# QEDProtocol/plonky2.5

Hardware: NVIDIA B200
Metric: commit Melem/s (2^20x135 LDE+Poseidon Merkle) (higher is better)
Workload: dtype u64 (Goldilocks field, integer + exact fp64 limb arithmetic)

## Files before the change

### plonky2.5_b200/csrc/gl_commit.cu

```cuda
#include <cuda_runtime.h>
#include <nvtx3/nvToolsExt.h>

#include <cstdio>
#include <algorithm>
#include <exception>
#include <cstring>
#include <cstdlib>
#include <condition_variable>
#include <map>
#include <thread>
#include <utility>
#include <memory>
#include <mutex>
#include <set>
#include <string>
#include <vector>

#include "../../include/gl_commit.h"
#include "fri.cuh"
#include "gates.cuh"
#include "merkle.cuh"
#include "microbench.cuh"
#include "ntt.cuh"
#include "ntt2.cuh"
#include "openings.cuh"
#include "peer_sync.cuh"
#include "permutation.cuh"

#ifndef LEAF_BLOCK
#define LEAF_BLOCK 128
#endif

namespace {

struct GlError {
    int code;
    std::string msg;
};

struct NvtxRange {
    explicit NvtxRange(const char* name) { nvtxRangePushA(name); }
    ~NvtxRange() { nvtxRangePop(); }
    NvtxRange(const NvtxRange&) = delete;
    NvtxRange& operator=(const NvtxRange&) = delete;
};


#define GL_THROW(code, ...)                              \
    do {                                                 \
        char _b[512];                                    \
        snprintf(_b, sizeof _b, __VA_ARGS__);            \
        throw GlError{code, _b};                         \
    } while (0)

#define CUDA_CHECK(expr)                                                                                   \
    do {                                                                                                   \
        cudaError_t _e = (expr);                                                                           \
        if (_e != cudaSuccess) {                                                                           \
            int _c = (_e == cudaErrorMemoryAllocation) ? GL_ERR_OOM : GL_ERR_CUDA;                         \
            GL_THROW(_c, "%s failed: %s (%s:%d)", #expr, cudaGetErrorString(_e), __FILE__, __LINE__);      \
        }                                                                                                  \
    } while (0)

struct DevPool {
    std::mutex mu;
    std::multimap<std::pair<int, size_t>, uint64_t*> free_list;
    size_t cached_words = 0;
    static DevPool& get() { static DevPool p; return p; }
    uint64_t* take(int dev, size_t words) {
        std::lock_guard<std::mutex> lk(mu);
        auto it = free_list.find({dev, words});
        if (it == free_list.end()) return nullptr;
        uint64_t* p = it->second;
        free_list.erase(it);
        cached_words -= words;
        return p;
    }
    void give(int dev, size_t words, uint64_t* p) {
        std::lock_guard<std::mutex> lk(mu);
        free_list.insert({{dev, words}, p});
        cached_words += words;
    }
    void trim(int dev) {
        std::lock_guard<std::mutex> lk(mu);
        for (auto it = free_list.begin(); it != free_list.end();) {
            if (it->first.first == dev) { cudaFree(it->second); cached_words -= it->first.second; it = free_list.erase(it); }
            else ++it;
        }
    }
};

struct DevBuf {
    uint64_t* p = nullptr;
    size_t words = 0;
    int dev = -1;
    void ensure(size_t w) {
        if (w <= words) return;
        release();
        if (w == 0) w = 1;
        CUDA_CHECK(cudaGetDevice(&dev));
        p = DevPool::get().take(dev, w);
        if (!p) {
            cudaError_t e = cudaMalloc(&p, w * sizeof(uint64_t));
            if (e == cudaErrorMemoryAllocation) {
                cudaGetLastError();
                DevPool::get().trim(dev);
                e = cudaMalloc(&p, w * sizeof(uint64_t));
            }
            if (e != cudaSuccess) { p = nullptr; CUDA_CHECK(e); }
        }
        words = w;
    }
    void release() {
        if (p && std::uncaught_exceptions() > 0) cudaDeviceSynchronize();
        if (p) DevPool::get().give(dev, words, p);
        p = nullptr;
        words = 0;
    }
    ~DevBuf() { release(); }
    DevBuf() = default;
    DevBuf(const DevBuf&) = delete;
    DevBuf& operator=(const DevBuf&) = delete;
};

inline uint32_t round_up(uint32_t x, uint32_t m) { return (x + m - 1) / m * m; }
inline uint32_t log2_exact(uint64_t n) {
    uint32_t l = 0;
    while ((1ULL << l) < n) l++;
    return l;
}
inline uint32_t h_bitrev(uint32_t x, uint32_t bits) {
    uint32_t r = 0;
    for (uint32_t i = 0; i < bits; i++) { r = (r << 1) | (x & 1); x >>= 1; }
    return r;
}

std::vector<uint32_t> plan_passes(uint32_t n, uint32_t max_a = 10) {
    std::vector<uint32_t> v;
    if (n < 3) return v;
    uint32_t k = (n + max_a - 1) / max_a, base = n / k, rem = n % k;
    for (uint32_t i = 0; i < k; i++) v.push_back(base + (i < rem ? 1 : 0));
    return v;
}

struct CosetTable {
    uint64_t g = 1;
    DevBuf F;
};

struct Tree {
    uint64_t n_leaves = 0;
    uint32_t leaf_len = 0, pitch = 0, cap_height = 0, degree_log = 0, rate_bits = 0;
    DevBuf leaves, digests, coeffs, d_cap;
    bool has_coeffs = false;
    std::vector<uint64_t> cap;
    Tree(uint64_t n_leaves_, uint32_t leaf_len_, uint32_t pitch_, uint32_t cap_height_)
        : n_leaves(n_leaves_), leaf_len(leaf_len_), pitch(pitch_), cap_height(cap_height_), cap(4ULL << cap_height_) {
        leaves.ensure(n_leaves * pitch);
        digests.ensure(n_digests() * 4);
        d_cap.ensure(4ULL << cap_height);
    }
    uint64_t n_digests() const { return 2 * (n_leaves - (1ULL << cap_height)); }
};

struct Fri {
    uint64_t len = 0;
    uint32_t rate_bits = 0, cap_height = 0;
    uint64_t shift = gl::COSET_SHIFT;
    uint32_t last_arity_bits = 0;
    DevBuf coeffs, values, tmp;
    Fri(uint64_t len_, uint32_t rate_bits_, uint32_t cap_height_) : len(len_), rate_bits(rate_bits_), cap_height(cap_height_) {
        coeffs.ensure(2 * len); values.ensure(2 * len); tmp.ensure(2 * len);
    }
};

struct Quotient {
    gl_handle wires = 0;
    uint64_t n_rows = 0;
    uint32_t n_challenges = 0;
    DevBuf acc, powers;
};

struct Openings {
    uint32_t log_n = 0;
    DevBuf final_poly, comp, refs, pw;
};

template <class T>
struct Handles {
    const char* kind;
    std::map<gl_handle, std::unique_ptr<T>> live;
    gl_handle put(gl_ctx* c, std::unique_ptr<T> obj);
    T* get(gl_handle h) const;
    void drop(gl_ctx* c, gl_handle h);
};

}

struct gl_ctx {
    int device = 0;
    cudaStream_t stream = nullptr;
    std::mutex mu;
    std::string err;
    std::map<uint32_t, std::unique_ptr<DevBuf>> roots;
    std::map<uint32_t, std::unique_ptr<DevBuf>> pass_roots;
    std::map<uint64_t, std::unique_ptr<std::vector<CosetTable>>> lde_tables;
    std::map<std::pair<uint64_t, uint32_t>, std::unique_ptr<CosetTable>> coset_cache;
    size_t coset_cache_words = 0;
    DevBuf in_stage, vals, scratch, hash_state;
    Handles<Tree> trees{"tree"};
    Handles<Fri> fris{"fri"};
    Handles<Openings> openings{"openings"};
    Handles<Quotient> quotients{"quotient"};
    float aux_ms = 0;
    gl_handle next_handle = 1;
    cudaStream_t copy_stream = nullptr;
    cudaStream_t send_stream = nullptr;
    cudaStream_t pull_stream = nullptr;
    cudaEvent_t ev_ntt[2] = {}, ev_sent[2] = {};
    bool sent_pending[2] = {false, false};
    DevBuf send_buf[2];
    std::set<const uint64_t*> own_ipc;
    bool trace = false;
    std::vector<cudaEvent_t> trace_ev;
    cudaEvent_t ev_sync = nullptr, ev_copyback = nullptr;
    std::vector<cudaEvent_t> chunk_ev, pull_ev, own_ev;
    DevBuf sync_err;
    cudaEvent_t ev[GL_N_STAGES + 1] = {};
    float stage_ms[GL_N_STAGES] = {};
    uint32_t launches[GL_N_STAGES] = {};
    int sm_count = 148;
};

namespace {

template <class T>
gl_handle Handles<T>::put(gl_ctx* c, std::unique_ptr<T> obj) {
    const gl_handle h = c->next_handle++;
    live[h] = std::move(obj);
    return h;
}
template <class T>
T* Handles<T>::get(gl_handle h) const {
    auto it = live.find(h);
    if (it == live.end()) GL_THROW(GL_ERR_HANDLE, "unknown %s handle %llu", kind, (unsigned long long)h);
    return it->second.get();
}
template <class T>
void Handles<T>::drop(gl_ctx* c, gl_handle h) {
    get(h);
    CUDA_CHECK(cudaStreamSynchronize(c->stream));
    live.erase(h);
}

const uint64_t* get_roots(gl_ctx* c, uint32_t log_n) {
    auto it = c->roots.find(log_n);
    if (it != c->roots.end()) return it->second->p;
    size_t half = log_n ? (size_t)1 << (log_n - 1) : 1;
    std::vector<uint64_t> w(half);
    uint64_t root = gl::h_root_of_unity(log_n), cur = 1;
    for (size_t e = 0; e < half; e++) { w[e] = cur; cur = gl::h_mul(cur, root); }
    auto buf = std::make_unique<DevBuf>();
    buf->ensure(half);
    CUDA_CHECK(cudaMemcpyAsync(buf->p, w.data(), half * 8, cudaMemcpyHostToDevice, c->stream));
    CUDA_CHECK(cudaStreamSynchronize(c->stream));
    const uint64_t* p = buf->p;
    c->roots[log_n] = std::move(buf);
    return p;
}

const uint64_t* get_pass_roots(gl_ctx* c, uint32_t a) {
    auto it = c->pass_roots.find(a);
    if (it != c->pass_roots.end()) return it->second->p;
    const size_t T = (size_t)1 << a, n = T;
    std::vector<uint64_t> w(n ? n : 1);
    uint64_t root = gl::h_root_of_unity(a), cur = 1;
    for (size_t e = 0; e < n; e++) {
        w[e] = e < (T >> 1) ? cur : gl::P - w[e - (T >> 1)];
        cur = gl::h_mul(cur, root);
    }
    auto buf = std::make_unique<DevBuf>();
    buf->ensure(w.size());
    CUDA_CHECK(cudaMemcpyAsync(buf->p, w.data(), w.size() * 8, cudaMemcpyHostToDevice, c->stream));
    CUDA_CHECK(cudaStreamSynchronize(c->stream));
    const uint64_t* p = buf->p;
    c->pass_roots[a] = std::move(buf);
    return p;
}

void fill_coset_table(gl_ctx* c, CosetTable& t, uint64_t g, uint32_t log_n) {
    t.g = g;
    if (log_n < 3) return;
    ntt::PowTable pt{};
    uint64_t sq = gl::canon(g);
    for (uint32_t k = 0; k < 32; k++) { pt.g2k[k] = sq; sq = gl::h_mul(sq, sq); }
    const uint64_t n = 1ULL << log_n;
    t.F.ensure(n);
    ntt::powers_kernel<<<(uint32_t)((n + 255) / 256), 256, 0, c->stream>>>(t.F.p, n, pt);
    CUDA_CHECK(cudaGetLastError());
}

const CosetTable* get_coset_table(gl_ctx* c, uint64_t g, uint32_t log_len) {
    auto key = std::make_pair(g, log_len);
    auto it = c->coset_cache.find(key);
    if (it != c->coset_cache.end()) return it->second.get();
    const size_t words = (size_t)1 << log_len;
    if (c->coset_cache_words + words > ((size_t)1 << 25)) {
        CUDA_CHECK(cudaStreamSynchronize(c->stream));
        c->coset_cache.clear();
        c->coset_cache_words = 0;
    }
    auto t = std::make_unique<CosetTable>();
    fill_coset_table(c, *t, g, log_len);
    c->coset_cache_words += words;
    const CosetTable* p = t.get();
    c->coset_cache[key] = std::move(t);
    return p;
}

const std::vector<CosetTable>& get_lde_tables(gl_ctx* c, uint32_t log_n, uint32_t rate_bits) {
    uint64_t key = ((uint64_t)log_n << 32) | rate_bits;
    auto it = c->lde_tables.find(key);
    if (it != c->lde_tables.end()) return *it->second;
    auto v = std::make_unique<std::vector<CosetTable>>((size_t)1 << rate_bits);
    uint64_t wR = gl::h_root_of_unity(log_n + rate_bits), g = gl::COSET_SHIFT;
    for (uint32_t s = 0; s < (1u << rate_bits); s++) {
        fill_coset_table(c, (*v)[s], g, log_n);
        g = gl::h_mul(g, wR);
    }
    auto& ref = *v;
    c->lde_tables[key] = std::move(v);
    return ref;
}

template <int G, int A>
void launch_pass_a(gl_ctx* c, const ntt::PassParams& p, uint32_t threads, size_t smem, uint32_t grid) {
    ntt::ntt_pass_kernel<G, A><<<grid, threads, smem, c->stream>>>(p);
}
template <int G, int A>
void prepare_pass2() {
    constexpr size_t smem = ntt2::smem_words<A, G>() * 8;
    if (smem > 48 * 1024) {
        static std::once_flag once[64];
        int dev = 0;
        CUDA_CHECK(cudaGetDevice(&dev));
        cudaError_t e = cudaSuccess;
        std::call_once(once[dev & 63], [&] { e = cudaFuncSetAttribute(ntt2::ntt_pass_kernel<G, A>, cudaFuncAttributeMaxDynamicSharedMemorySize, (int)smem); });
        CUDA_CHECK(e);
    }
}
template <int G, int A>
void launch_pass2_a(gl_ctx* c, const ntt::PassParams& p, uint32_t grid) {
    constexpr size_t smem = ntt2::smem_words<A, G>() * 8;
    constexpr uint32_t threads = (1u << A) * G / 16;
    prepare_pass2<G, A>();
    ntt2::ntt_pass_kernel<G, A><<<grid, threads, smem, c->stream>>>(p);
}

template <int G, int A>
void preload_pass2() {
    cudaFuncAttributes at;
    CUDA_CHECK(cudaFuncGetAttributes(&at, ntt2::ntt_pass_kernel<G, A>));
    prepare_pass2<G, A>();
    if constexpr (A > 3) preload_pass2<G, A - 1>();
}
void preload_stream_kernels() {
    static std::once_flag once[64];
    int dev = 0;
    CUDA_CHECK(cudaGetDevice(&dev));
    cudaError_t e = cudaSuccess;
    std::call_once(once[dev & 63], [&] {
        cudaFuncAttributes at;
        auto load = [&](const void* f) { if (e == cudaSuccess) e = cudaFuncGetAttributes(&at, f); };
        load((const void*)ntt::transpose_in_kernel);
        load((const void*)ntt::ntt_tiny_kernel);
        load((const void*)peersync::signal_kernel);
        load((const void*)peersync::wait_kernel);
        load((const void*)merkle::leaf_absorb_kernel<LEAF_BLOCK>);
        load((const void*)merkle::tree_level_kernel<128>);
    });
    CUDA_CHECK(e);
    preload_pass2<4, 10>();
    preload_pass2<8, 10>();
}
template <int G>
void launch_pass2(gl_ctx* c, ntt::PassParams p, uint32_t cols_padded, uint32_t* launches) {
    p.ncg = cols_padded / G;
    const uint64_t grid = (uint64_t)p.ncg << (p.log_n - p.a);
    if (grid >= (1ULL << 31)) GL_THROW(GL_ERR_UNSUPPORTED, "NTT grid too large");
    switch (p.a) {
        case 3: launch_pass2_a<G, 3>(c, p, (uint32_t)grid); break;
        case 4: launch_pass2_a<G, 4>(c, p, (uint32_t)grid); break;
        case 5: launch_pass2_a<G, 5>(c, p, (uint32_t)grid); break;
        case 6: launch_pass2_a<G, 6>(c, p, (uint32_t)grid); break;
        case 7: launch_pass2_a<G, 7>(c, p, (uint32_t)grid); break;
        case 8: launch_pass2_a<G, 8>(c, p, (uint32_t)grid); break;
        case 9: launch_pass2_a<G, 9>(c, p, (uint32_t)grid); break;
        case 10: launch_pass2_a<G, 10>(c, p, (uint32_t)grid); break;
        default: GL_THROW(GL_ERR_INVALID, "run_ntt: pass size %u has no second-generation kernel", p.a);
    }
    CUDA_CHECK(cudaGetLastError());
    if (launches) (*launches)++;
}

template <int G>
void launch_pass(gl_ctx* c, ntt::PassParams p, uint32_t cols_padded, uint32_t* launches) {
    p.ncg = cols_padded / G;
    uint32_t T = 1u << p.a;
    uint32_t threads = T * G / 8;
    size_t smem = ((size_t)(T + (T >> 3)) * G + (T - (T >> 3))) * 8;
    uint64_t grid = (uint64_t)p.ncg << (p.log_n - p.a);
    if (grid >= (1ULL << 31)) GL_THROW(GL_ERR_UNSUPPORTED, "NTT grid too large");
    if constexpr (G == 2) {
        launch_pass_a<G, 0>(c, p, threads, smem, (uint32_t)grid);
    } else {
        switch (p.a) {
            case 3: launch_pass_a<G, 3>(c, p, threads, smem, (uint32_t)grid); break;
            case 4: launch_pass_a<G, 4>(c, p, threads, smem, (uint32_t)grid); break;
            case 5: launch_pass_a<G, 5>(c, p, threads, smem, (uint32_t)grid); break;
            case 6: launch_pass_a<G, 6>(c, p, threads, smem, (uint32_t)grid); break;
            case 7: launch_pass_a<G, 7>(c, p, threads, smem, (uint32_t)grid); break;
            case 8: launch_pass_a<G, 8>(c, p, threads, smem, (uint32_t)grid); break;
            case 9: launch_pass_a<G, 9>(c, p, threads, smem, (uint32_t)grid); break;
            case 10:
                if constexpr (G == 4) { launch_pass_a<G, 10>(c, p, threads, smem, (uint32_t)grid); break; }
                [[fallthrough]];
            default: GL_THROW(GL_ERR_INVALID, "bad pass size %u", p.a);
        }
    }
    CUDA_CHECK(cudaGetLastError());
    if (launches) (*launches)++;
}

void run_ntt(gl_ctx* c, uint64_t* src, uint32_t src_pitch, uint64_t* dst, uint32_t dst_pitch, uint32_t cols_padded,
             uint32_t log_n, bool ifft, const CosetTable* pre, int G, uint32_t* launches, const ntt::Scatter* scatter = nullptr,
             const uint64_t* const* src_list = nullptr) {
    if (src_list && (ifft || scatter || (G != 4 && G != 8) || log_n < 3 || cols_padded / G > (uint32_t)ntt::MAX_PEERS))
        GL_THROW(GL_ERR_INVALID, "run_ntt: unsupported multi-source transform");
    const uint64_t* W = get_roots(c, log_n);
    uint64_t n_inv = ifft ? gl::h_inv(((uint64_t)1 << log_n) % gl::P) : 1;
    auto passes = plan_passes(log_n, 10);
    if (passes.empty()) {
        dim3 grid((cols_padded + 63) / 64, 1u << log_n);
        ntt::ntt_tiny_kernel<<<grid, 64, 0, c->stream>>>(src, dst, src_pitch, dst_pitch, cols_padded, log_n,
                                                         gl::h_root_of_unity(log_n), pre ? pre->g : 1, scatter ? 2 : (ifft ? 1 : 0), n_inv,
                                                         scatter ? *scatter : ntt::Scatter{});
        CUDA_CHECK(cudaGetLastError());
        if (launches) (*launches)++;
        return;
    }
    uint32_t log_blk = log_n;
    for (size_t i = 0; i < passes.size(); i++) {
        bool first = i == 0, last = i + 1 == passes.size();
        ntt::PassParams p{};
        p.log_n = log_n;
        p.log_blk = log_blk;
        p.a = passes[i];
        p.W = W;
        p.Wa = get_pass_roots(c, passes[i]);
        p.pre = (first && pre) ? pre->F.p : nullptr;
        p.store_mode = (ifft && last) ? 1 : 0;
        p.scale = (ifft && last) ? n_inv : 1;
        if (scatter && last) {
            p.store_mode = 2;
            memcpy(p.peer, scatter->peer, sizeof p.peer);
            p.scatter_row0 = scatter->row0; p.log_rows_per_peer = scatter->log_rows_per_peer;
            p.scatter_col0 = scatter->col0; p.scatter_pitch = scatter->pitch; p.scatter_ncols = scatter->ncols;
        }
        if (ifft) {
            p.src = src; p.src_pitch = src_pitch;
            p.dst = last ? dst : src; p.dst_pitch = last ? dst_pitch : src_pitch;
        } else {
            p.src = first ? src : dst; p.src_pitch = first ? src_pitch : dst_pitch;
            p.dst = dst; p.dst_pitch = dst_pitch;
        }
        const bool aligned = p.src_pitch % 2 == 0 && p.dst_pitch % 2 == 0 && ((uintptr_t)p.src % 16 == 0) && ((uintptr_t)p.dst % 16 == 0);
        if (src_list) {
            int g = G;
            if (first) {
                p.src_list = 1; p.src = nullptr; p.src_pitch = (uint32_t)G;
                for (uint32_t k = 0; k < cols_padded / G; k++) {
                    if ((uintptr_t)src_list[k] % 16) GL_THROW(GL_ERR_INVALID, "run_ntt: misaligned source block");
                    p.peer[k] = const_cast<uint64_t*>(src_list[k]);
                }
            } else if (cols_padded % 8 == 0) {
                g = 8;
            }
            if (p.dst_pitch % 2 || (uintptr_t)p.dst % 16) GL_THROW(GL_ERR_INVALID, "run_ntt: misaligned destination");
            g == 8 ? launch_pass2<8>(c, p, cols_padded, launches) : launch_pass2<4>(c, p, cols_padded, launches);
        } else if ((G == 8 || G == 4) && aligned) {
            G == 8 ? launch_pass2<8>(c, p, cols_padded, launches) : launch_pass2<4>(c, p, cols_padded, launches);
        } else {
            switch (G) {
                case 8:
                    p.a == 10 ? launch_pass<4>(c, p, cols_padded, launches) : launch_pass<8>(c, p, cols_padded, launches);
                    break;
                case 4: launch_pass<4>(c, p, cols_padded, launches); break;
                case 2: launch_pass<2>(c, p, cols_padded, launches); break;
                default: GL_THROW(GL_ERR_INVALID, "bad column group");
            }
        }
        log_blk -= passes[i];
    }
}

void merkle_levels(gl_ctx* c, uint64_t n_leaves, uint32_t cap_height, uint64_t* d_digests, uint64_t* d_cap, uint32_t* tree_launches) {
    const uint32_t log_sub = log2_exact(n_leaves) - cap_height;
    for (uint32_t layer = 1; layer <= log_sub; layer++) {
        uint64_t n_nodes = n_leaves >> layer;
        constexpr int TB = 128;
        merkle::tree_level_kernel<TB><<<(uint32_t)((n_nodes + TB - 1) / TB), TB, 0, c->stream>>>(d_digests, d_cap, layer, log_sub, n_nodes);
        CUDA_CHECK(cudaGetLastError());
        if (tree_launches) (*tree_launches)++;
    }
}

void merkle_build(gl_ctx* c, const uint64_t* d_leaves, uint64_t n_leaves, uint32_t leaf_len, uint32_t pitch,
                  uint32_t cap_height, uint64_t* d_digests, uint64_t* d_cap, uint32_t* leaf_launches,
                  uint32_t* tree_launches, cudaEvent_t after_leaves) {
    NvtxRange nv("build Merkle tree");
    uint32_t log_leaves = log2_exact(n_leaves);
    uint32_t log_sub = log_leaves - cap_height;
    constexpr int LB = LEAF_BLOCK;
    merkle::leaf_hash_kernel<LB><<<(uint32_t)((n_leaves + LB - 1) / LB), LB, 0, c->stream>>>(
        d_leaves, pitch, leaf_len, n_leaves, log_sub, d_digests, d_cap);
    CUDA_CHECK(cudaGetLastError());
    if (leaf_launches) (*leaf_launches)++;
    if (after_leaves) CUDA_CHECK(cudaEventRecord(after_leaves, c->stream));
    merkle_levels(c, n_leaves, cap_height, d_digests, d_cap, tree_launches);
}

void leaf_absorb(gl_ctx* c, const uint64_t* d_leaves, uint64_t n_leaves, uint32_t leaf_len, uint32_t pitch, uint32_t cap_height, uint32_t col0,
                 uint32_t col1, uint64_t* d_state, uint64_t* d_digests, uint64_t* d_cap, bool first, bool last, uint32_t* leaf_launches) {
    const uint32_t log_sub = log2_exact(n_leaves) - cap_height;
    constexpr int LB = LEAF_BLOCK;
    merkle::leaf_absorb_kernel<LB><<<(uint32_t)((n_leaves + LB - 1) / LB), LB, 0, c->stream>>>(d_leaves, pitch, leaf_len, col0, col1, n_leaves, log_sub,
                                                                                             d_state, d_digests, d_cap, first ? 1 : 0, last ? 1 : 0);
    CUDA_CHECK(cudaGetLastError());
    if (leaf_launches) (*leaf_launches)++;
}

void check_shape(uint32_t n_cols, uint32_t log_n, uint32_t rate_bits, uint32_t cap_height) {
    if (n_cols == 0) GL_THROW(GL_ERR_INVALID, "empty polynomial batch");
    if (log_n + rate_bits > 31) GL_THROW(GL_ERR_UNSUPPORTED, "log_n + rate_bits = %u > 31", log_n + rate_bits);
    if (cap_height > log_n + rate_bits)
        GL_THROW(GL_ERR_INVALID, "cap_height should be at most log2(leaves.len()) (cap_height=%u, log2(leaves)=%u)",
                 cap_height, log_n + rate_bits);
}

void finish_tree(gl_ctx* c, std::unique_ptr<Tree> t, uint64_t* out_digests, uint64_t* out_cap, gl_handle* out_tree) {
    CUDA_CHECK(cudaMemcpyAsync(t->cap.data(), t->d_cap.p, t->cap.size() * 8, cudaMemcpyDeviceToHost, c->stream));
    if (out_digests && t->n_digests())
        CUDA_CHECK(cudaMemcpyAsync(out_digests, t->digests.p, t->n_digests() * 32, cudaMemcpyDeviceToHost, c->stream));
    CUDA_CHECK(cudaStreamSynchronize(c->stream));
    memcpy(out_cap, t->cap.data(), t->cap.size() * 8);
    if (out_tree) *out_tree = c->trees.put(c, std::move(t));
}

void copy_row(gl_ctx* c, const Tree* t, uint64_t row, uint64_t* out_row) {
    CUDA_CHECK(cudaMemcpyAsync(out_row, t->leaves.p + row * t->pitch, (size_t)t->leaf_len * 8, cudaMemcpyDeviceToHost, c->stream));
    CUDA_CHECK(cudaStreamSynchronize(c->stream));
}

void record(gl_ctx* c, int i) { CUDA_CHECK(cudaEventRecord(c->ev[i], c->stream)); }

void reset_stages(gl_ctx* c, int first, int end) {
    for (int i = first; i < end; i++) { c->launches[i] = 0; c->stage_ms[i] = 0; }
// ... 1914 lines not shown
```

### plonky2.5_b200/csrc/ntt2.cuh

```cuda
#pragma once
#include "ntt.cuh"

namespace ntt2 {

struct W3 { uint32_t l, h, t; };

__device__ __forceinline__ W3 w3(uint64_t x) { return {(uint32_t)x, (uint32_t)(x >> 32), 0u}; }

__device__ __forceinline__ W3 add3(const W3 a, const W3 b) {
    W3 r;
    asm("add.cc.u32  %0, %3, %6;\n\t"
        "addc.cc.u32 %1, %4, %7;\n\t"
        "addc.u32    %2, %5, %8;"
        : "=&r"(r.l), "=&r"(r.h), "=r"(r.t) : "r"(a.l), "r"(a.h), "r"(a.t), "r"(b.l), "r"(b.h), "r"(b.t));
    return r;
}
__device__ __forceinline__ W3 sub3(const W3 a, const W3 b) {
    W3 r;
    asm("sub.cc.u32  %0, %3, %6;\n\t"
        "subc.cc.u32 %1, %4, %7;\n\t"
        "subc.u32    %2, %5, %8;"
        : "=&r"(r.l), "=&r"(r.h), "=r"(r.t) : "r"(a.l), "r"(a.h), "r"(a.t), "r"(b.l), "r"(b.h), "r"(b.t));
    return r;
}
template <uint32_t K>
__device__ __forceinline__ W3 bias3(const W3 a) {
    W3 r;
    asm("add.cc.u32  %0, %3, %6;\n\t"
        "addc.cc.u32 %1, %4, %7;\n\t"
        "addc.u32    %2, %5, %8;"
        : "=&r"(r.l), "=&r"(r.h), "=r"(r.t) : "r"(a.l), "r"(a.h), "r"(a.t), "n"(K), "n"(0u - K), "n"(K - 1));
    return r;
}
__device__ __forceinline__ uint64_t fold3(const W3 a) {
    uint32_t l, h;
    asm("{\n\t.reg .u32 u0, u1, c;\n\t"
        "sub.cc.u32  u0, 0, %4;\n\t"
        "subc.u32    u1, %4, 0;\n\t"
        "add.cc.u32  %0, %2, u0;\n\t"
        "addc.cc.u32 %1, %3, u1;\n\t"
        "addc.u32    c, 0, 0;\n\t"
        "neg.s32     c, c;\n\t"
        "add.cc.u32  %0, %0, c;\n\t"
        "addc.u32    %1, %1, 0;\n\t"
        "}" : "=&r"(l), "=&r"(h) : "r"(a.l), "r"(a.h), "r"(a.t));
    return ((uint64_t)h << 32) | l;
}
__device__ __forceinline__ uint64_t reduce3(uint32_t z0, uint32_t z1, uint32_t z2) {
    uint32_t l, h;
    asm("{\n\t.reg .u32 d, ds;\n\t"
        "sub.cc.u32  %0, %2, %4;\n\t"
        "subc.cc.u32 %1, %3, 0;\n\t"
        "subc.u32    d, 0, 0;\n\t"
        "add.cc.u32  %1, %1, %4;\n\t"
        "addc.u32    d, d, 0;\n\t"
        "shr.s32     ds, d, 31;\n\t"
        "sub.cc.u32  %0, %0, d;\n\t"
        "subc.u32    %1, %1, ds;\n\t"
        "add.u32     %1, %1, d;\n\t"
        "}" : "=&r"(l), "=&r"(h) : "r"(z0), "r"(z1), "r"(z2));
    return ((uint64_t)h << 32) | l;
}
template <int S>
__device__ __forceinline__ uint64_t shift_mul(const W3 a) {
    constexpr int R = S % 32, W = S / 32;
    static_assert(R > 0 && W <= 2, "unsupported shift");
    const uint32_t y0 = a.l << R, y1 = __funnelshift_l(a.l, a.h, R), y2 = __funnelshift_l(a.h, a.t, R);
    if (W == 0) return reduce3(y0, y1, y2);
    if (W == 1) return gl::reduce_words(0u, y0, y1, y2);
    uint32_t r0, r1, r2, r3;
    asm("sub.cc.u32  %0, 0, %4;\n\t"
        "subc.cc.u32 %1, %4, %5;\n\t"
        "subc.cc.u32 %2, %5, %6;\n\t"
        "subc.u32    %3, %6, 0;"
        : "=&r"(r0), "=&r"(r1), "=&r"(r2), "=r"(r3) : "r"(y0), "r"(y1), "r"(y2));
    return gl::reduce_words(r0, r1, r2, r3);
}

__device__ __forceinline__ void dft8_cs(W3 (&x)[8], uint64_t (&out)[8]) {
    x[0] = bias3<22>(x[0]); x[2] = bias3<5>(x[2]); x[5] = bias3<10>(x[5]); x[7] = bias3<5>(x[7]);
    W3 a[8];
    a[0] = add3(x[0], x[4]); a[4] = sub3(x[0], x[4]);
    a[1] = add3(x[1], x[5]); a[5] = w3(shift_mul<24>(sub3(x[5], x[1])));
    a[2] = add3(x[2], x[6]); a[6] = w3(shift_mul<48>(sub3(x[2], x[6])));
    a[3] = add3(x[3], x[7]); a[7] = w3(shift_mul<72>(sub3(x[7], x[3])));
    a[5] = bias3<2>(a[5]);
    W3 b[8];
    b[0] = add3(a[0], a[2]); b[2] = sub3(a[0], a[2]);
    b[1] = add3(a[1], a[3]); b[3] = w3(shift_mul<48>(sub3(a[1], a[3])));
    b[4] = add3(a[4], a[6]); b[6] = sub3(a[4], a[6]);
    b[5] = add3(a[5], a[7]); b[7] = w3(shift_mul<48>(sub3(a[5], a[7])));
    out[0] = fold3(add3(b[0], b[1])); out[1] = fold3(sub3(b[0], b[1]));
    out[2] = fold3(add3(b[2], b[3])); out[3] = fold3(sub3(b[2], b[3]));
    out[4] = fold3(add3(b[4], b[5])); out[5] = fold3(sub3(b[4], b[5]));
    out[6] = fold3(add3(b[6], b[7])); out[7] = fold3(sub3(b[6], b[7]));
}
__device__ __forceinline__ void dft8_cs(uint64_t (&x)[8]) {
    W3 v[8];
#pragma unroll
    for (int j = 0; j < 8; j++) v[j] = w3(x[j]);
    dft8_cs(v, x);
}

__device__ __forceinline__ void dft16_cs(uint64_t (&x)[16]) {
    W3 s[8], d[8];
    {
        const W3 x0 = bias3<2>(w3(x[0])), x8 = w3(x[8]);
        s[0] = add3(x0, x8); d[0] = sub3(x0, x8);
    }
#define NTT2_PAIR(J, SH, NEG)                                                                        \
    {                                                                                                \
        W3 lo = w3(x[J]), hi = w3(x[J + 8]);                                                         \
        if (NEG) { hi = bias3<2>(hi); s[J] = add3(lo, hi); d[J] = w3(shift_mul<SH>(sub3(hi, lo))); } \
        else { lo = bias3<2>(lo); s[J] = add3(lo, hi); d[J] = w3(shift_mul<SH>(sub3(lo, hi))); }     \
    }
    NTT2_PAIR(1, 60, true) NTT2_PAIR(2, 24, true) NTT2_PAIR(3, 84, false) NTT2_PAIR(4, 48, false)
    NTT2_PAIR(5, 12, false) NTT2_PAIR(6, 72, true) NTT2_PAIR(7, 36, true)
#undef NTT2_PAIR
    uint64_t lo8[8], hi8[8];
    dft8_cs(s, lo8);
    dft8_cs(d, hi8);
#pragma unroll
    for (int j = 0; j < 8; j++) { x[j] = lo8[j]; x[j + 8] = hi8[j]; }
}

__device__ __forceinline__ void mbar_init(uint64_t* bar, uint32_t count) {
    asm volatile("mbarrier.init.shared::cta.b64 [%0], %1;" ::"r"((uint32_t)__cvta_generic_to_shared(bar)), "r"(count));
    asm volatile("fence.mbarrier_init.release.cluster;" ::: "memory");
}
__device__ __forceinline__ void tma_bulk_g2s(void* smem_dst, const void* gmem_src, uint32_t bytes, uint64_t* bar) {
    const uint32_t b = (uint32_t)__cvta_generic_to_shared(bar);
    asm volatile("mbarrier.arrive.expect_tx.shared::cta.b64 _, [%0], %1;" ::"r"(b), "r"(bytes) : "memory");
    asm volatile("cp.async.bulk.shared::cluster.global.mbarrier::complete_tx::bytes [%0], [%1], %2, [%3];"
                 ::"r"((uint32_t)__cvta_generic_to_shared(smem_dst)), "l"(gmem_src), "r"(bytes), "r"(b) : "memory");
}
__device__ __forceinline__ void mbar_wait(uint64_t* bar, uint32_t parity) {
    const uint32_t b = (uint32_t)__cvta_generic_to_shared(bar);
    asm volatile("{\n\t.reg .pred p;\n\t"
                 "WAIT_%=:\n\t"
                 "mbarrier.try_wait.parity.shared::cta.b64 p, [%0], %1;\n\t"
                 "@p bra DONE_%=;\n\t"
                 "bra WAIT_%=;\n\t"
                 "DONE_%=:\n\t}" ::"r"(b), "r"(parity) : "memory");
}

__host__ __device__ constexpr int plan_n(int A) { return A >= 9 ? 3 : (A >= 5 ? 2 : 1); }
__host__ __device__ constexpr int plan_k(int A, int r) {
    switch (A) {
        case 3: return r == 0 ? 3 : 0;
        case 4: return r == 0 ? 4 : 0;
        case 5: return r == 0 ? 3 : (r == 1 ? 2 : 0);
        case 6: return r < 2 ? 3 : 0;
        case 7: return r == 0 ? 3 : (r == 1 ? 4 : 0);
        case 8: return r < 2 ? 4 : 0;
        case 9: return r < 3 ? 3 : 0;
        case 10: return r < 2 ? 3 : (r == 2 ? 4 : 0);
        default: return 0;
    }
}

__device__ __forceinline__ uint32_t insk(uint32_t q, uint32_t sh, uint32_t e, uint32_t k) {
    return ((q >> sh) << (sh + k)) | (e << sh) | (q & ((1u << sh) - 1));
}
__host__ __device__ constexpr uint32_t brev_const(uint32_t e, int k) {
    uint32_t r = 0;
    for (int i = 0; i < k; i++) r |= ((e >> i) & 1u) << (k - 1 - i);
    return r;
}

template <int A>
__host__ __device__ constexpr int pad_shift() { return plan_k(A, plan_n(A) - 1) == 4 ? 4 : 3; }
template <int A, int G>
__host__ __device__ constexpr size_t smem_words() { return (size_t)((1u << A) + ((1u << A) >> pad_shift<A>())) * G + (1u << A); }

__device__ __forceinline__ uint64_t inter_twiddle(const ntt::PassParams& p, uint32_t l, uint32_t a, uint32_t o_lo) {
    const uint32_t N = 1u << p.log_n;
    const uint32_t ex = (o_lo * gl::bitrev32(l, a)) << (p.log_n - p.log_blk);
    return ex >= (N >> 1) ? gl::P - __ldg(p.W + (ex - (N >> 1))) : __ldg(p.W + ex);
}
__device__ __forceinline__ uint64_t finish(const ntt::PassParams& p, uint64_t v, uint64_t w, uint32_t b_lo) {
    if (b_lo) v = gl::mul(v, w);
    if (p.scale != 1) v = gl::mul(v, p.scale);
    if (!b_lo) v = gl::canon(v);
    return v;
}
__device__ __forceinline__ uint64_t* dest(const ntt::PassParams& p, uint32_t prow, uint32_t col) {
    if (p.store_mode == 2) {
        const uint64_t grow = p.scatter_row0 + prow;
        return p.peer[grow >> p.log_rows_per_peer] + (grow & ((1ULL << p.log_rows_per_peer) - 1)) * p.scatter_pitch + p.scatter_col0 + col;
    }
    const uint32_t N = 1u << p.log_n;
    const uint32_t drow = p.store_mode == 1 ? ((N - gl::bitrev32(prow, p.log_n)) & (N - 1)) : prow;
    return p.dst + (uint64_t)drow * p.dst_pitch + col;
}

template <int G, int A>
__global__ void __launch_bounds__((1 << A) * G / 16 >= 32 ? (1 << A) * G / 16 : 32,
                                   (1 << A) * G / 16 >= 32 ? 1024 / ((1 << A) * G / 16) : 32)
ntt_pass_kernel(const ntt::PassParams p) {
    constexpr int NR = plan_n(A);
    constexpr uint32_t T = 1u << A, G2 = G / 2, PAD = pad_shift<A>();
    extern __shared__ __align__(128) uint64_t sm2[];
    __shared__ uint64_t wl_bar;
    uint64_t* tile = sm2;
    uint64_t* Wl = sm2 + (size_t)(T + (T >> PAD)) * G;
    const uint32_t tid = threadIdx.x;
    const uint32_t cg = blockIdx.x % p.ncg, tile_id = blockIdx.x / p.ncg;
    const uint32_t b_lo = p.log_blk - A;
    const uint32_t o_lo = tile_id & ((1u << b_lo) - 1), o_hi = tile_id >> b_lo;
    const uint32_t row_base = (o_hi << p.log_blk) | o_lo;
    auto phys = [](uint32_t l) { return l + (l >> PAD); };
    const uint32_t q8 = tid / G2, c2 = tid % G2, q16 = tid / G, c1 = tid % G;
    const uint32_t col2 = cg * G + 2 * c2, col1 = cg * G + c1;
    const uint64_t* const src = p.src_list ? p.peer[cg] - (size_t)cg * G : p.src;

    if (NR > 1) {
        if (tid == 0) mbar_init(&wl_bar, 1);
        __syncthreads();
    }
    ulonglong2 v[8];
    uint64_t u[16];
    constexpr int K0 = plan_k(A, 0);
    constexpr uint32_t SH0 = A - K0;
    {
        if (K0 == 3) {
#pragma unroll
            for (int e = 0; e < 8; e++) {
                const uint64_t row = row_base | ((uint64_t)insk(q8, SH0, e, 3) << b_lo);
                v[e] = *reinterpret_cast<const ulonglong2*>(src + row * p.src_pitch + col2);
            }
        } else {
#pragma unroll
            for (int e = 0; e < 16; e++) {
                const uint64_t row = row_base | ((uint64_t)insk(q16, SH0, e, 4) << b_lo);
                u[e] = src[row * p.src_pitch + col1];
            }
        }
    }
    if (NR > 1 && tid == 0) tma_bulk_g2s(Wl, p.Wa, T * 8, &wl_bar);
    if (p.pre != nullptr) {
        if (K0 == 3) {
#pragma unroll
            for (int e = 0; e < 8; e++) {
                const uint64_t row = row_base | ((uint64_t)insk(q8, SH0, e, 3) << b_lo);
                const uint64_t g = __ldg(p.pre + row);
                v[e].x = gl::mul(v[e].x, g);
                v[e].y = gl::mul(v[e].y, g);
            }
        } else {
#pragma unroll
            for (int e = 0; e < 16; e++) {
                const uint64_t row = row_base | ((uint64_t)insk(q16, SH0, e, 4) << b_lo);
                u[e] = gl::mul(u[e], __ldg(p.pre + row));
            }
        }
    }
    if (NR > 1) mbar_wait(&wl_bar, 0);

    int done = 0;
#pragma unroll
    for (int r = 0; r < NR; r++) {
        const int k = plan_k(A, r);
        const uint32_t sh = A - done - k;
        const bool last = r + 1 == NR;
        if (r > 0) {
            const int kp = plan_k(A, r - 1);
            const uint32_t shp = A - done;
            {
                if (kp == 3) {
#pragma unroll
                    for (int e = 0; e < 8; e++)
                        *reinterpret_cast<ulonglong2*>(tile + (size_t)phys(insk(q8, shp, e, 3)) * G + 2 * c2) = v[e];
                } else {
#pragma unroll
                    for (int e = 0; e < 16; e++) tile[(size_t)phys(insk(q16, shp, e, 4)) * G + c1] = u[e];
                }
            }
            __syncthreads();
            {
                if (k == 4) {
#pragma unroll
                    for (int e = 0; e < 16; e++) u[e] = tile[(size_t)phys(insk(q16, sh, e, 4)) * G + c1];
                } else {
#pragma unroll
                    for (int e = 0; e < 8; e++)
                        v[e] = *reinterpret_cast<const ulonglong2*>(tile + (size_t)phys(insk(q8, k == 3 ? sh : 0, e, 3)) * G + 2 * c2);
                }
            }
            if (!last) __syncthreads();
        }
        {
            if (k == 4) {
                dft16_cs(u);
                if (!last) {
                    const uint32_t step = (q16 & ((1u << sh) - 1)) << (A - sh - 4);
#pragma unroll
                    for (int e = 1; e < 16; e++) u[e] = gl::mul(u[e], Wl[step * brev_const(e, 4)]);
                }
            } else if (k == 3) {
                uint64_t x[8], y[8];
#pragma unroll
                for (int e = 0; e < 8; e++) { x[e] = v[e].x; y[e] = v[e].y; }
                dft8_cs(x);
                dft8_cs(y);
                if (!last) {
                    const uint32_t step = (q8 & ((1u << sh) - 1)) << (A - sh - 3);
#pragma unroll
                    for (int e = 1; e < 8; e++) {
                        const uint64_t w = Wl[step * brev_const(e, 3)];
                        x[e] = gl::mul(x[e], w);
                        y[e] = gl::mul(y[e], w);
                    }
                }
#pragma unroll
                for (int e = 0; e < 8; e++) v[e] = make_ulonglong2(x[e], y[e]);
            } else {
                uint64_t x[8], y[8];
#pragma unroll
                for (int e = 0; e < 8; e++) { x[e] = v[e].x; y[e] = v[e].y; }
                ntt::radix8_round(x, Wl, A, 0, 0, 2);
                ntt::radix8_round(y, Wl, A, 0, 0, 2);
#pragma unroll
                for (int e = 0; e < 8; e++) v[e] = make_ulonglong2(x[e], y[e]);
            }
        }
        done += k;
    }
    constexpr int KL = plan_k(A, NR - 1);
    if (KL == 4) {
        if (p.store_mode == 0 && p.scale == 1) {
            uint64_t* d = p.dst + (uint64_t)(row_base | ((q16 << 4) << b_lo)) * p.dst_pitch + col1;
            const uint64_t stride = (uint64_t)p.dst_pitch << b_lo;
            if (b_lo == 0) {
#pragma unroll
                for (int e = 0; e < 16; e++) d[e * stride] = gl::canon(u[e]);
            } else {
                const uint32_t N = 1u << p.log_n, sh = p.log_n - p.log_blk;
                constexpr uint32_t A4 = A >= 4 ? A - 4 : 0;
                const uint32_t ex0 = (o_lo * gl::bitrev32(q16, A4)) << sh, exs = (o_lo << A4) << sh;
#pragma unroll
                for (int e = 0; e < 16; e++) {
                    const uint32_t ex = ex0 + exs * brev_const(e, 4);
                    const uint64_t w = ex >= (N >> 1) ? gl::P - __ldg(p.W + (ex - (N >> 1))) : __ldg(p.W + ex);
                    d[e * stride] = gl::mul(u[e], w);
                }
            }
            return;
        }
#pragma unroll
        for (int e = 0; e < 16; e++) {
            const uint32_t l = insk(q16, 0, e, 4);
            const uint64_t val = finish(p, u[e], b_lo ? inter_twiddle(p, l, A, o_lo) : 1, b_lo);
            if (p.store_mode == 2 && col1 >= p.scatter_ncols) continue;
            *dest(p, row_base | (l << b_lo), col1) = val;
        }
    } else {
#pragma unroll
        for (int e = 0; e < 8; e++) {
            const uint32_t l = insk(q8, 0, e, 3);
            const uint64_t w = b_lo ? inter_twiddle(p, l, A, o_lo) : 1;
            ulonglong2 val;
            val.x = finish(p, v[e].x, w, b_lo);
            val.y = finish(p, v[e].y, w, b_lo);
            uint64_t* d = dest(p, row_base | (l << b_lo), col2);
            if (p.store_mode == 2) {
                if (col2 + 1 < p.scatter_ncols && ((p.scatter_col0 | p.scatter_pitch) & 1) == 0) *reinterpret_cast<ulonglong2*>(d) = val;
                else {
                    if (col2 < p.scatter_ncols) d[0] = val.x;
                    if (col2 + 1 < p.scatter_ncols) d[1] = val.y;
                }
            } else {
                *reinterpret_cast<ulonglong2*>(d) = val;
            }
        }
    }
}

}
```

Baseline: 1257.

## Use full root table, mad-based Goldilocks reductions in NTT pass kernel

Result: no change. 1266, median of 6 (+0.7%).

```diff
diff --git a/plonky2.5_b200/csrc/gl_commit.cu b/plonky2.5_b200/csrc/gl_commit.cu
--- a/plonky2.5_b200/csrc/gl_commit.cu
+++ b/plonky2.5_b200/csrc/gl_commit.cu
@@ -256,13 +256,14 @@
 const uint64_t* get_roots(gl_ctx* c, uint32_t log_n) {
     auto it = c->roots.find(log_n);
     if (it != c->roots.end()) return it->second->p;
-    size_t half = log_n ? (size_t)1 << (log_n - 1) : 1;
-    std::vector<uint64_t> w(half);
-    uint64_t root = gl::h_root_of_unity(log_n), cur = 1;
-    for (size_t e = 0; e < half; e++) { w[e] = cur; cur = gl::h_mul(cur, root); }
+    const uint64_t n = 1ULL << log_n;
+    ntt::PowTable pt{};
+    uint64_t sq = gl::h_root_of_unity(log_n);
+    for (uint32_t k = 0; k < 32; k++) { pt.g2k[k] = sq; sq = gl::h_mul(sq, sq); }
     auto buf = std::make_unique<DevBuf>();
-    buf->ensure(half);
-    CUDA_CHECK(cudaMemcpyAsync(buf->p, w.data(), half * 8, cudaMemcpyHostToDevice, c->stream));
+    buf->ensure(n);
+    ntt::powers_kernel<<<(uint32_t)((n + 255) / 256), 256, 0, c->stream>>>(buf->p, n, pt);
+    CUDA_CHECK(cudaGetLastError());
     CUDA_CHECK(cudaStreamSynchronize(c->stream));
     const uint64_t* p = buf->p;
     c->roots[log_n] = std::move(buf);
diff --git a/plonky2.5_b200/csrc/ntt2.cuh b/plonky2.5_b200/csrc/ntt2.cuh
--- a/plonky2.5_b200/csrc/ntt2.cuh
+++ b/plonky2.5_b200/csrc/ntt2.cuh
@@ -34,47 +34,50 @@
 }
 __device__ __forceinline__ uint64_t fold3(const W3 a) {
     uint32_t l, h;
-    asm("{\n\t.reg .u32 u0, u1, c;\n\t"
-        "sub.cc.u32  u0, 0, %4;\n\t"
-        "subc.u32    u1, %4, 0;\n\t"
-        "add.cc.u32  %0, %2, u0;\n\t"
-        "addc.cc.u32 %1, %3, u1;\n\t"
-        "addc.u32    c, 0, 0;\n\t"
-        "neg.s32     c, c;\n\t"
-        "add.cc.u32  %0, %0, c;\n\t"
-        "addc.u32    %1, %1, 0;\n\t"
+    asm("{\n\t.reg .u32 c;\n\t"
+        "mad.lo.cc.u32  %0, %4, 0xFFFFFFFF, %2;\n\t"
+        "madc.hi.cc.u32 %1, %4, 0xFFFFFFFF, %3;\n\t"
+        "addc.u32       c, 0, 0;\n\t"
+        "mad.lo.cc.u32  %0, c, 0xFFFFFFFF, %0;\n\t"
+        "madc.hi.u32    %1, c, 0xFFFFFFFF, %1;\n\t"
         "}" : "=&r"(l), "=&r"(h) : "r"(a.l), "r"(a.h), "r"(a.t));
     return ((uint64_t)h << 32) | l;
 }
-__device__ __forceinline__ uint64_t reduce3(uint32_t z0, uint32_t z1, uint32_t z2) {
+__device__ __forceinline__ uint64_t reduce4(uint32_t z0, uint32_t z1, uint32_t z2, uint32_t z3) {
     uint32_t l, h;
     asm("{\n\t.reg .u32 d, ds;\n\t"
-        "sub.cc.u32  %0, %2, %4;\n\t"
-        "subc.cc.u32 %1, %3, 0;\n\t"
-        "subc.u32    d, 0, 0;\n\t"
-        "add.cc.u32  %1, %1, %4;\n\t"
-        "addc.u32    d, d, 0;\n\t"
-        "shr.s32     ds, d, 31;\n\t"
-        "sub.cc.u32  %0, %0, d;\n\t"
-        "subc.u32    %1, %1, ds;\n\t"
-        "add.u32     %1, %1, d;\n\t"
-        "}" : "=&r"(l), "=&r"(h) : "r"(z0), "r"(z1), "r"(z2));
+        "mad.lo.cc.u32  %0, %4, 0xFFFFFFFF, %2;\n\t"
+        "madc.hi.cc.u32 %1, %4, 0xFFFFFFFF, %3;\n\t"
+        "addc.u32       d, 0, 0;\n\t"
+        "sub.cc.u32     %0, %0, %5;\n\t"
+        "subc.cc.u32    %1, %1, 0;\n\t"
+        "subc.u32       d, d, 0;\n\t"
+        "shr.s32        ds, d, 31;\n\t"
+        "sub.cc.u32     %0, %0, d;\n\t"
+        "subc.u32       %1, %1, ds;\n\t"
+        "add.u32        %1, %1, d;\n\t"
+        "}" : "=&r"(l), "=&r"(h) : "r"(z0), "r"(z1), "r"(z2), "r"(z3));
     return ((uint64_t)h << 32) | l;
+}
+__device__ __forceinline__ uint64_t mul(uint64_t a, uint64_t b) {
+    uint32_t z0, z1, z2, z3;
+    gl::mul_words_c(a, b, z0, z1, z2, z3);
+    return reduce4(z0, z1, z2, z3);
 }
 template <int S>
 __device__ __forceinline__ uint64_t shift_mul(const W3 a) {
     constexpr int R = S % 32, W = S / 32;
     static_assert(R > 0 && W <= 2, "unsupported shift");
     const uint32_t y0 = a.l << R, y1 = __funnelshift_l(a.l, a.h, R), y2 = __funnelshift_l(a.h, a.t, R);
-    if (W == 0) return reduce3(y0, y1, y2);
-    if (W == 1) return gl::reduce_words(0u, y0, y1, y2);
+    if (W == 0) return fold3({y0, y1, y2});
+    if (W == 1) return reduce4(0u, y0, y1, y2);
     uint32_t r0, r1, r2, r3;
     asm("sub.cc.u32  %0, 0, %4;\n\t"
         "subc.cc.u32 %1, %4, %5;\n\t"
         "subc.cc.u32 %2, %5, %6;\n\t"
         "subc.u32    %3, %6, 0;"
         : "=&r"(r0), "=&r"(r1), "=&r"(r2), "=r"(r3) : "r"(y0), "r"(y1), "r"(y2));
-    return gl::reduce_words(r0, r1, r2, r3);
+    return reduce4(r0, r1, r2, r3);
 }
 
 __device__ __forceinline__ void dft8_cs(W3 (&x)[8], uint64_t (&out)[8]) {
@@ -174,13 +177,12 @@
 __host__ __device__ constexpr size_t smem_words() { return (size_t)((1u << A) + ((1u << A) >> pad_shift<A>())) * G + (1u << A); }
 
 __device__ __forceinline__ uint64_t inter_twiddle(const ntt::PassParams& p, uint32_t l, uint32_t a, uint32_t o_lo) {
-    const uint32_t N = 1u << p.log_n;
     const uint32_t ex = (o_lo * gl::bitrev32(l, a)) << (p.log_n - p.log_blk);
-    return ex >= (N >> 1) ? gl::P - __ldg(p.W + (ex - (N >> 1))) : __ldg(p.W + ex);
+    return __ldg(p.W + ex);
 }
 __device__ __forceinline__ uint64_t finish(const ntt::PassParams& p, uint64_t v, uint64_t w, uint32_t b_lo) {
-    if (b_lo) v = gl::mul(v, w);
-    if (p.scale != 1) v = gl::mul(v, p.scale);
+    if (b_lo) v = mul(v, w);
+    if (p.scale != 1) v = mul(v, p.scale);
     if (!b_lo) v = gl::canon(v);
     return v;
 }
@@ -244,14 +246,14 @@
             for (int e = 0; e < 8; e++) {
                 const uint64_t row = row_base | ((uint64_t)insk(q8, SH0, e, 3) << b_lo);
                 const uint64_t g = __ldg(p.pre + row);
-                v[e].x = gl::mul(v[e].x, g);
-                v[e].y = gl::mul(v[e].y, g);
+                v[e].x = mul(v[e].x, g);
+                v[e].y = mul(v[e].y, g);
             }
         } else {
 #pragma unroll
             for (int e = 0; e < 16; e++) {
                 const uint64_t row = row_base | ((uint64_t)insk(q16, SH0, e, 4) << b_lo);
-                u[e] = gl::mul(u[e], __ldg(p.pre + row));
+                u[e] = mul(u[e], __ldg(p.pre + row));
             }
         }
     }
@@ -295,7 +297,7 @@
                 if (!last) {
                     const uint32_t step = (q16 & ((1u << sh) - 1)) << (A - sh - 4);
 #pragma unroll
-                    for (int e = 1; e < 16; e++) u[e] = gl::mul(u[e], Wl[step * brev_const(e, 4)]);
+                    for (int e = 1; e < 16; e++) u[e] = mul(u[e], Wl[step * brev_const(e, 4)]);
                 }
             } else if (k == 3) {
                 uint64_t x[8], y[8];
@@ -308,8 +310,8 @@
 #pragma unroll
                     for (int e = 1; e < 8; e++) {
                         const uint64_t w = Wl[step * brev_const(e, 3)];
-                        x[e] = gl::mul(x[e], w);
-                        y[e] = gl::mul(y[e], w);
+                        x[e] = mul(x[e], w);
+                        y[e] = mul(y[e], w);
                     }
                 }
 #pragma unroll
@@ -335,14 +337,13 @@
 #pragma unroll
                 for (int e = 0; e < 16; e++) d[e * stride] = gl::canon(u[e]);
             } else {
-                const uint32_t N = 1u << p.log_n, sh = p.log_n - p.log_blk;
+                const uint32_t sh = p.log_n - p.log_blk;
                 constexpr uint32_t A4 = A >= 4 ? A - 4 : 0;
                 const uint32_t ex0 = (o_lo * gl::bitrev32(q16, A4)) << sh, exs = (o_lo << A4) << sh;
 #pragma unroll
                 for (int e = 0; e < 16; e++) {
                     const uint32_t ex = ex0 + exs * brev_const(e, 4);
-                    const uint64_t w = ex >= (N >> 1) ? gl::P - __ldg(p.W + (ex - (N >> 1))) : __ldg(p.W + ex);
-                    d[e * stride] = gl::mul(u[e], w);
+                    d[e * stride] = mul(u[e], __ldg(p.W + ex));
                 }
             }
             return;
```
